# Gardlin/PCR-CG

Hardware: AMD Instinct MI355X
Metric: fragment-pairs/s KPFCNN+GCN fwd, 30k-pt pairs (higher is better)
Workload: dtype f32

## Files before the change

include/pcrcg.h:

```cpp
#ifndef PCRCG_H
#define PCRCG_H

#include <stddef.h>
#include <stdint.h>

#ifdef __cplusplus
extern "C" {
#endif

#define PCRCG_OK 0
#define PCRCG_EBADARG (-1)
#define PCRCG_EWORKSPACE (-2)
#define PCRCG_ELAUNCH (-3)
#define PCRCG_ECAPACITY (-4)

#define PCRCG_KPOINTS 15

const char* pcrcg_last_error(void);
#define PCRCG_ABI_VERSION 4
int pcrcg_abi_version(void);

int pcrcg_debug_set(const char* spec);
int pcrcg_debug_release(void);

// ... 6 lines not shown
int pcrcg_umap_order(const uint64_t* keys, int m, int* order, void* ws, size_t ws_bytes, void* stream);

size_t pcrcg_cellgrid_ws_bytes(int ns, int nb);
int pcrcg_cellgrid_build(const float* sup, int ns, const int* slen, int nb, float radius, void* grid,
                         size_t grid_bytes, void* stream);
int pcrcg_radius_query(const float* q, int nq, const int* qlen, int ns, const int* slen, int nb,
                       float radius, const void* grid, int cols, int64_t* out_idx, int* out_count,
                       int* out_max_count, int* status, void* stream);
int pcrcg_radius_query_ex(const float* q, int nq, const int* qlen, int ns, const int* slen, int nb,
                          float radius, const void* grid, int cols, int64_t* out_idx, int* out_count,
                          int* out_max_count, int* status, int* out_tie_rows, int* out_tie_count, void* stream);
int pcrcg_radius_query_groups(const float* q, int nq, const int* qlen, int ns, const int* slen, int nb, int group,
                              float radius, const void* grid, int cols, int64_t* out_idx, int* out_count,
                              int* out_max_count, int* status, int* out_tie_rows, int* out_tie_count, void* stream);
int pcrcg_radius_query_cells(const void* qgrid, const float* q, int nq, const int* qlen, const void* sgrid, int ns,
                             const int* slen, int nb, int group, float radius, int cols, int64_t* out_idx, int* out_count,
                             int* out_max_count, int* status, int* out_tie_rows, int* out_tie_count, void* stream);
size_t pcrcg_radius_neighbors_ws_bytes(int ns, int nb);
int pcrcg_radius_neighbors_batch(const float* q, int nq, const float* sup, int ns, const int* qlen,
                                 const int* slen, int nb, float radius, int cols, int64_t* out_idx,
                                 int* out_count, int* out_max_count, int* status, void* ws,
                                 size_t ws_bytes, void* stream);

#define PCRCG_MAX_REORDER_JOBS 12
typedef struct pcrcg_reorder_job {
    const float* q;
    const int* qlen;
    const int* rows;
    const int* count;
    int64_t* idx;
    int nq, nbq, cloud0, nrows, max_count, cols;
    float radius;
    int group;
    const float* sup;
    const void* forest;
    int forest_ns, forest_nb;
} pcrcg_reorder_job;
size_t pcrcg_kdforest_ws_bytes(int ns, int nb);
int pcrcg_kdforest_build(const float* sup, int ns, const int* slen, int nb, void* forest, size_t forest_bytes,
                         void* stream);
int pcrcg_radius_reorder(const float* q, int nq, const int* qlen, int nbq, const float* sup, int ns, int nb,
                         const void* forest, int cloud0, float radius, const int* rows, int nrows, const int* count,
                         int max_count, int cols, int64_t* idx, int* status, void* stream);
int pcrcg_radius_reorder_jobs(const pcrcg_reorder_job* jobs, int njobs, const float* sup, int ns, int nb,
                              const void* forest, int* status, void* stream);

size_t pcrcg_kpconv_ws_bytes(int ns);
int pcrcg_kpconv_aggregate(const float* q_pts, int nq, const float* s_pts, int ns, const int64_t* idx,
                           int h, int ld_idx, const float* x, int cin, const float* kp, float extent,
                           float* wf, float* inv_n, void* ws, size_t ws_bytes, void* stream);
int pcrcg_kpconv_aggregate_bf16(const float* q_pts, int nq, const float* s_pts, int ns, const int64_t* idx, int h,
                                int ld_idx, const float* x, int cin, const float* kp, float extent, void* x_bf16,
                                void* wf_bf16, float* inv_n, void* ws, size_t ws_bytes, void* stream);

void pcrcg_profile_kpconv(int enable);
int pcrcg_profile_kpconv_read(float* ms, int* nq, int* h, int* cin, int* cout, int* kind, int cap);

int pcrcg_gemm_f32(const float* a, int lda, const float* b, int ldb, int trans_b, float* c, int ldc, int m,
                   int n, int k, const float* row_scale, const float* bias, void* stream);
size_t pcrcg_gemm_colstats_bytes(int m, int n);
int pcrcg_gemm_f32_colstats(const float* a, int lda, const float* b, int ldb, int trans_b, float* c, int ldc,
                            int m, int n, int k, const float* row_scale, const float* bias, void* colstats,
                            size_t colstats_bytes, int* h_chunks, void* stream);
int pcrcg_gemm_bf16a_f32_colstats(const void* a_bf16, int lda, const float* b, int ldb, float* c, int ldc, int m, int n,
                                  int k, const float* row_scale, const float* bias, void* colstats,
                                  size_t colstats_bytes, int* h_chunks, void* stream);

int pcrcg_gemm_f32_fused(const float* a, int lda, const int64_t* idx, int ld_idx, int ns, const float* zero_row,
                         const void* a_sums, double a_count, float a_eps, float a_slope, const float* b, int ldb,
                         const float* bias, float* c, int ldc, int m, int n, int k, int accumulate, void* stream);

void pcrcg_gemm_set_mode(int mode);
int pcrcg_gemm_get_mode(void);
int pcrcg_gemm_redo_counts(unsigned long long* out2, int reset);
void pcrcg_thread_shares_gpu(int on);

int pcrcg_gather_max(const float* x, int ns, int c, const int64_t* idx, int nq, int h, int ld_idx,
                     float* out, void* stream);
int pcrcg_gather_first(const float* x, int ns, int c, const int64_t* idx, int nq, int ld_idx, float* out,
                       int ld_out, void* stream);
size_t pcrcg_instnorm_ws_bytes(int c);
int pcrcg_instnorm_stats_from_partials(const void* partials, int chunks, int c, double count, float eps,
                                       float* stats, void* stream);
int pcrcg_instnorm_stats(const float* x, int n, int c, int ldx, float eps, float* stats, void* ws,
                         size_t ws_bytes, void* stream);
int pcrcg_instnorm_apply(const float* x, int n, int c, int ldx, const float* stats, const float* res,
                         int ldr, const float* res_stats, float slope, float* y, int ldy, void* stream);
int pcrcg_instnorm_colsums(const float* x, int n, int c, int ldx, void* sums, void* stream);
int pcrcg_instnorm_apply_sums(const float* x, int n, int c, int ldx, const void* sums, double count, float eps,
                              const float* res, int ldr, const void* res_sums, float slope, float* y, int ldy,
                              void* stream);

int pcrcg_fill2d(float* dst, int ld, int rows, int cols, float value, void* stream);
int pcrcg_inject_image_features(const float* fmap, int c, int h, int w, const float* valid, const int64_t* inds2d,
                                const int64_t* inds3d, int n, long row_offset, long n_rows, float* x, int ldx,
                                void* stream);

typedef struct pcrcg_image_frame {
    const float* fmap;
    const float* depth;
    const float* valid;
    float world2camera[16];
    float intrinsics[16];
    float thresh;
    int h, w;
    int depth_h, depth_w;
// ... 191 lines not shown
```

pcrcg_amd/_lib.py:

```python
import ctypes
import os

_HERE = os.path.dirname(os.path.abspath(__file__))
LIB_PATH = os.path.join(_HERE, "libpcrcg_hip.so")


def lib_identity():
    import hashlib
    with open(LIB_PATH, "rb") as f:
        return LIB_PATH, hashlib.sha256(f.read()).hexdigest()[:16]

ABI_VERSION = 4

c_int, c_float, c_void_p, c_size_t = ctypes.c_int, ctypes.c_float, ctypes.c_void_p, ctypes.c_size_t

SIGNATURES = {
    "pcrcg_last_error": (ctypes.c_char_p, []),
    "pcrcg_abi_version": (c_int, []),
    "pcrcg_debug_set": (c_int, [ctypes.c_char_p]),
    "pcrcg_check_status": (c_int, [c_void_p, c_void_p]),
    "pcrcg_grid_subsample_ws_bytes": (c_size_t, [c_int, c_int]),
    "pcrcg_grid_subsample_batch": (c_int, [c_void_p, c_int, c_void_p, c_int, c_float, c_int, c_void_p, c_void_p,
                                           c_void_p, c_void_p, c_size_t, c_void_p]),
    "pcrcg_umap_order_ws_bytes": (c_size_t, [c_int]),
    "pcrcg_umap_order": (c_int, [c_void_p, c_int, c_void_p, c_void_p, c_size_t, c_void_p]),
    "pcrcg_cellgrid_ws_bytes": (c_size_t, [c_int, c_int]),
    "pcrcg_cellgrid_build": (c_int, [c_void_p, c_int, c_void_p, c_int, c_float, c_void_p, c_size_t, c_void_p]),
    "pcrcg_radius_query": (c_int, [c_void_p, c_int, c_void_p, c_int, c_void_p, c_int, c_float, c_void_p, c_int,
                                   c_void_p, c_void_p, c_void_p, c_void_p, c_void_p]),
    "pcrcg_radius_query_ex": (c_int, [c_void_p, c_int, c_void_p, c_int, c_void_p, c_int, c_float, c_void_p, c_int,
                                      c_void_p, c_void_p, c_void_p, c_void_p, c_void_p, c_void_p, c_void_p]),
    "pcrcg_radius_query_groups": (c_int, [c_void_p, c_int, c_void_p, c_int, c_void_p, c_int, c_int, c_float, c_void_p, c_int,
                                          c_void_p, c_void_p, c_void_p, c_void_p, c_void_p, c_void_p, c_void_p]),
    "pcrcg_radius_query_cells": (c_int, [c_void_p, c_void_p, c_int, c_void_p, c_void_p, c_int, c_void_p, c_int, c_int, c_float,
                                         c_int, c_void_p, c_void_p, c_void_p, c_void_p, c_void_p, c_void_p, c_void_p]),
    "pcrcg_kdforest_ws_bytes": (c_size_t, [c_int, c_int]),
    "pcrcg_kdforest_build": (c_int, [c_void_p, c_int, c_void_p, c_int, c_void_p, c_size_t, c_void_p]),
    "pcrcg_radius_reorder": (c_int, [c_void_p, c_int, c_void_p, c_int, c_void_p, c_int, c_int, c_void_p, c_int,
                                     c_float, c_void_p, c_int, c_void_p, c_int, c_int, c_void_p, c_void_p, c_void_p]),
    "pcrcg_radius_reorder_jobs": (c_int, [c_void_p, c_int, c_void_p, c_int, c_int, c_void_p, c_void_p, c_void_p]),
    "pcrcg_radius_neighbors_ws_bytes": (c_size_t, [c_int, c_int]),
    "pcrcg_radius_neighbors_batch": (c_int, [c_void_p, c_int, c_void_p, c_int, c_void_p, c_void_p, c_int, c_float,
                                             c_int, c_void_p, c_void_p, c_void_p, c_void_p, c_void_p, c_size_t,
                                             c_void_p]),
    "pcrcg_kpconv_ws_bytes": (c_size_t, [c_int]),
    "pcrcg_kpconv_aggregate": (c_int, [c_void_p, c_int, c_void_p, c_int, c_void_p, c_int, c_int, c_void_p, c_int,
                                       c_void_p, c_float, c_void_p, c_void_p, c_void_p, c_size_t, c_void_p]),
    "pcrcg_kpconv_aggregate_bf16": (c_int, [c_void_p, c_int, c_void_p, c_int, c_void_p, c_int, c_int, c_void_p, c_int,
                                            c_void_p, c_float, c_void_p, c_void_p, c_void_p, c_void_p, c_size_t,
                                            c_void_p]),
    "pcrcg_profile_kpconv": (None, [c_int]),
    "pcrcg_profile_kpconv_read": (c_int, [c_void_p, c_void_p, c_void_p, c_void_p, c_void_p, c_void_p, c_int]),
    "pcrcg_gemm_f32": (c_int, [c_void_p, c_int, c_void_p, c_int, c_int, c_void_p, c_int, c_int, c_int, c_int,
                               c_void_p, c_void_p, c_void_p]),
    "pcrcg_gemm_colstats_bytes": (c_size_t, [c_int, c_int]),
    "pcrcg_gemm_f32_colstats": (c_int, [c_void_p, c_int, c_void_p, c_int, c_int, c_void_p, c_int, c_int, c_int, c_int,
                                        c_void_p, c_void_p, c_void_p, c_size_t, c_void_p, c_void_p]),
    "pcrcg_gemm_bf16a_f32_colstats": (c_int, [c_void_p, c_int, c_void_p, c_int, c_void_p, c_int, c_int, c_int, c_int,
                                              c_void_p, c_void_p, c_void_p, c_size_t, c_void_p, c_void_p]),
    "pcrcg_gemm_f32_fused": (c_int, [c_void_p, c_int, c_void_p, c_int, c_int, c_void_p, c_void_p, ctypes.c_double, c_float,
                                     c_float, c_void_p, c_int, c_void_p, c_void_p, c_int, c_int, c_int, c_int, c_int, c_void_p]),
    "pcrcg_gemm_set_mode": (None, [c_int]),
    "pcrcg_gemm_get_mode": (c_int, []),
    "pcrcg_gemm_redo_counts": (c_int, [c_void_p, c_int]),
    "pcrcg_instnorm_stats_from_partials": (c_int, [c_void_p, c_int, c_int, ctypes.c_double, c_float, c_void_p,
                                                   c_void_p]),
    "pcrcg_gather_max": (c_int, [c_void_p, c_int, c_int, c_void_p, c_int, c_int, c_int, c_void_p, c_void_p]),
    "pcrcg_gather_first": (c_int, [c_void_p, c_int, c_int, c_void_p, c_int, c_int, c_void_p, c_int, c_void_p]),
    "pcrcg_instnorm_ws_bytes": (c_size_t, [c_int]),
    "pcrcg_instnorm_stats": (c_int, [c_void_p, c_int, c_int, c_int, c_float, c_void_p, c_void_p, c_size_t, c_void_p]),
    "pcrcg_instnorm_apply": (c_int, [c_void_p, c_int, c_int, c_int, c_void_p, c_void_p, c_int, c_void_p, c_float,
                                     c_void_p, c_int, c_void_p]),
    "pcrcg_instnorm_colsums": (c_int, [c_void_p, c_int, c_int, c_int, c_void_p, c_void_p]),
    "pcrcg_instnorm_apply_sums": (c_int, [c_void_p, c_int, c_int, c_int, c_void_p, ctypes.c_double, c_float, c_void_p, c_int,
                                          c_void_p, c_float, c_void_p, c_int, c_void_p]),
    "pcrcg_fill2d": (c_int, [c_void_p, c_int, c_int, c_int, c_float, c_void_p]),
    "pcrcg_inject_image_features": (c_int, [c_void_p, c_int, c_int, c_int, c_void_p, c_void_p, c_void_p, c_int, ctypes.c_long,
                                            ctypes.c_long, c_void_p, c_int, c_void_p]),
    "pcrcg_project_depth_ws_bytes": (c_size_t, [c_int]),
    "pcrcg_project_depth": (c_int, [c_void_p, c_int, c_void_p, c_int, c_int, c_void_p, c_void_p, c_float, c_void_p, c_void_p,
                                    c_void_p, c_void_p, c_size_t, c_void_p]),
    "pcrcg_inject_frames": (c_int, [c_void_p, ctypes.c_long, ctypes.c_long, c_void_p, c_int, c_int, c_void_p, c_int, c_void_p]),
    "pcrcg_superglue_valid_maps": (c_int, [c_void_p, c_int, c_void_p, c_int, c_void_p, c_void_p, c_int, c_int, c_int, c_void_p,
                                           c_void_p, c_void_p]),
    "pcrcg_knn": (c_int, [c_void_p, c_int, c_int, c_void_p, c_void_p]),
    "pcrcg_edgeconv_ws_bytes": (c_size_t, [c_int]),
    "pcrcg_edgeconv_reduce": (c_int, [c_void_p, c_int, c_void_p, c_int, c_void_p, c_int, c_int, c_int, c_float,
                                      c_void_p, c_int, c_void_p, c_void_p, c_size_t, c_void_p]),
    "pcrcg_edgeconv_reduce_sums": (c_int, [c_void_p, c_int, c_void_p, c_int, c_void_p, c_int, c_int, c_int, c_void_p, c_int,
                                           c_void_p, c_void_p]),
    "pcrcg_softmax_rows": (c_int, [c_void_p, c_int, c_int, c_int, c_float, c_void_p]),
    "pcrcg_attention_supported": (c_int, [c_int]),
    "pcrcg_attention": (c_int, [c_void_p, c_int, c_void_p, c_int, c_void_p, c_int, c_void_p, c_int, c_int, c_int, c_int,
                                c_int, c_float, c_void_p]),
    "pcrcg_softmax_matvec": (c_int, [c_void_p, c_int, c_int, c_int, c_float, c_void_p, c_int, c_void_p, c_int, c_void_p]),
    "pcrcg_copy2d": (c_int, [c_void_p, c_int, c_void_p, c_int, c_int, c_int, c_void_p]),
    "pcrcg_add": (c_int, [c_void_p, c_void_p, c_void_p, ctypes.c_long, c_void_p]),
    "pcrcg_l2norm_rows": (c_int, [c_void_p, c_int, c_void_p, c_int, c_int, c_int, c_void_p]),
    "pcrcg_sigmoid_scores": (c_int, [c_void_p, c_int, c_void_p, c_int, c_void_p]),
    "pcrcg_kpfcnn_ws_bytes": (c_size_t, [c_void_p, c_void_p]),
    "pcrcg_kpfcnn_group_ws_bytes": (c_size_t, [c_void_p, c_void_p, c_int]),
    "pcrcg_kpfcnn_forward_group": (c_int, [c_void_p, c_void_p, c_void_p, c_int, c_void_p, c_size_t, c_void_p]),
    "pcrcg_kpfcnn_forward": (c_int, [c_void_p, c_void_p, c_void_p, c_void_p, c_size_t, c_void_p]),
# ... 111 lines not shown
```

pcrcg_amd/csrc/common.h:

```cpp
#pragma once
#include <hip/hip_runtime.h>

#include <cstdarg>
#include <cstdint>
#include <cstdio>
#include <mutex>

#include "pcrcg.h"

namespace pcrcg {

void set_error(const char* fmt, ...);

inline hipStream_t as_stream(void* s) { return reinterpret_cast<hipStream_t>(s); }

struct Carver {
    char* base;
    size_t cap;
    size_t off = 0;
    Carver(void* ws, size_t bytes) : base(static_cast<char*>(ws)), cap(bytes) {}
    template <typename T>
    T* take(size_t count) {
        size_t bytes = (count * sizeof(T) + 255) & ~size_t(255);
        T* p = reinterpret_cast<T*>(base + off);
// ... 20 lines not shown
void gemm_x6_release_det();
void trainops_release_det();
void conv2d_release_det();

int kdforest_build_levels(const float* sup, int ns, const int* slen, int nb, int per_level, const int* level_base, void* forest,
                          size_t forest_bytes, hipStream_t stream);

int radius_fast_cap();
int radius_query_pass(const float* q, int nq, const int* qlen, int ns, const int* slen, int nb, int group, float radius,
                      const void* grid, int cols, int64_t* out_idx, int* out_count, int* out_max_count, int* status,
                      int* out_tie_rows, int* out_tie_count, hipStream_t st, int pass);

bool gemm_x6_shared();
void gemm_x6_set_shared(int on);
int radius_cells_pass(const void* qgrid, const float* q, int nq, const int* qlen, const void* sgrid, int ns, const int* slen,
                      int nb, int group, float radius, int cols, int64_t* out_idx, int* out_count, int* out_max_count,
                      int* status, int* out_tie_rows, int* out_tie_count, hipStream_t st, int pass);
constexpr int kRadiusRedoStatus = 4;

struct GemmExtra {
    const long long* a_idx = nullptr;
    int a_idx_ld = 0, a_ns = 0;
    const float* a_zero = nullptr;
    bool accumulate = false;
    const double* a_sums = nullptr;
    double a_count = 0.0;
    float a_eps = 1e-5f, a_slope = 1.0f;
    int grad_operand = 0;
};

struct GemmPair {
    const float* a = nullptr;
    float* c = nullptr;
    int m = 0;
    const float* row_scale = nullptr;
    void* colstats = nullptr;
    int* h_chunks = nullptr;
    bool c_zeroed = false;
    const long long* a_idx = nullptr;
    int a_ns = 0;
    const double* a_sums = nullptr;
    double a_count = 0.0;
};
struct GemmGroup {
    int n = 0;
    GemmPair p[3];
};

int kpconv_pack(const float* x, int ns, int cin, const float* s_pts, void* ws, size_t ws_bytes, hipStream_t st,
                unsigned short* x_bf16 = nullptr);
int kpconv_aggregate_rows(const float* q_pts, int nq, const float* s_pts, int ns, const int64_t* idx, int h, int ld_idx,
                          const float* x, int cin, const float* kp, float extent, float* wf, float* inv_n, void* ws,
                          size_t ws_bytes, hipStream_t st, bool pack, bool stream_out, int c1_ld = 0);
int kpconv_aggregate_bf16(const float* q_pts, int nq, const float* s_pts, int ns, const int64_t* idx, int h, int ld_idx,
                          const float* x, unsigned short* x_bf16, int cin, const float* kp, float extent,
                          unsigned short* wf_bf16, float* inv_n, void* ws, size_t ws_bytes, hipStream_t st);

struct NormJob {
    const float* x; const double* sums; const float* res; const double* res_sums; float* y;
    const float* s_pts; float4* pk;
    int n; double count;
    float* stats_out = nullptr;
};
int instnorm_apply_sums_multi(const NormJob* jobs, int count, int c, int ldx, float eps, int ldr, float slope, int ldy, bool pack,
                              hipStream_t st);

struct GatherJob { const float* x; const int64_t* idx; float* out; int ns, nq, h, ld_idx; };
int gather_max_multi(const GatherJob* jobs, int count, int c, hipStream_t st);
int heads_multi(const float* const* x, const int* rows, int count, int ld, int fd, float* const* feats, float* const* s_ov,
                float* const* s_sal, hipStream_t st);
int copy2d_multi(const float* const* src, float* const* dst, const int* rows, int count, int ld_src, int ld_dst, int cols,
                 hipStream_t st);
int instnorm_colsums_multi(const float* const* x, double* const* sums, const int* n, int count, int c, int ldx, hipStream_t st);

struct EdgeCloud {
    const float* ctr; const float* nbr; const int* idx; float* emax; double* sums; int n, k;
};
bool edgeconv_rows_ok(const EdgeCloud* cl, int count, int ld_ctr, int ld_nbr, int ld_emax, int c);
int edgeconv_rows_multi(const EdgeCloud* cl, int count, int ld_ctr, int ld_nbr, int ld_emax, int c, bool atomic, int* nchunks_out,
                        hipStream_t st);

struct AttnCloud { const float* q; const float* k; const float* v; float* out; int n, ms; };
bool attention_mfma_ok(const AttnCloud* cl, int count, int ldq, int ldk, int ldv, int d);
int attention_mfma_multi(const AttnCloud* cl, int count, int ldq, int ldk, int ldv, int ldo, int heads, int d, float scale,
                         hipStream_t st);
bool attention_bwd_mfma_ok(int n, int ms, int d, int ldq, int ldk, int ldv, int ld_do);
int attention_bwd_mfma(const float* q, int ldq, const float* k, int ldk, const float* v, int ldv, const float* o, int ldo,
                       const float* d_o, int ld_do, float* dq, int ld_dq, float* dk, int ld_dk, float* dv, int ld_dv, int n, int ms,
                       int heads, int d, float scale, hipStream_t st);

struct DebugOpts {
    int stat_sums = 1;
    int stat_sums_rows = 1 << 30;
    int att_mfma = 1;
    int radius_blocks = 0;
    int kd_blocks = 0;
    int att_tq = 16;
    int kd_spin_limit = 0;
    int gemm_log = 0;
    int x6_tile = -1, x6_splitk = 0, x6_t1 = 1, x6_t2 = 1, x6_order = -1, x6_big = 0, x6_h2 = 1;
    int train_side_stream = 1;
    int gemm_tile = -1, gemm_splitk = 0, gemm_split_target = 768;
    int deterministic = 0;
    int bwd_mfma = 1;
};
const DebugOpts& debug_opts();
// ... 63 lines not shown
```

pcrcg_amd/csrc/kpconv.hip:

```cpp
#include <mutex>
#include <vector>

#include <hip/hip_ext.h>

#include "common.h"

namespace pcrcg {

struct ProfRec { hipEvent_t a, b; int nq, h, cin, cout, kind; };
static int g_prof_on = 0;
static std::vector<ProfRec> g_prof;
static std::mutex g_prof_mu;

KpProfScope::KpProfScope(hipStream_t s, int nq_, int h_, int cin_, int cout_, int kind_)
    : st(s), a(nullptr), b(nullptr), nq(nq_), h(h_), cin(cin_), cout(cout_), kind(kind_),
      on((g_prof_on & (kind_ == 3 ? 2 : kind_ == 4 ? 4 : 1)) != 0) {
    if (!on) return;
    (void)hipEventCreate(&a);
    (void)hipEventCreate(&b);
}
KpProfScope::~KpProfScope() {
    if (!on) return;
    std::lock_guard<std::mutex> lock(g_prof_mu);
    g_prof.push_back({a, b, nq, h, cin, cout, kind});
// ... 183 lines not shown
    float kpx[K], kpy[K], kpz[K];
#pragma unroll
    for (int k = 0; k < K; ++k) { kpx[k] = kp[3 * k]; kpy[k] = kp[3 * k + 1]; kpz[k] = kp[3 * k + 2]; }
    const float inv_extent = 1.0f / extent;
    const float qx = q_pts[3 * (long)q], qy = q_pts[3 * (long)q + 1], qz = q_pts[3 * (long)q + 2];
    float acc[K];
#pragma unroll
    for (int k = 0; k < K; ++k) acc[k] = 0.f;
    int npos = 0;
    const long long* row = idx + (long)q * ld_idx;
    for (int h0 = 0; h0 < H; h0 += C1_PARTS * C1_BATCH) {
        long long iv[C1_BATCH];
#pragma unroll
        for (int b = 0; b < C1_BATCH; ++b) {
            const int h = h0 + b * C1_PARTS + part;
            iv[b] = row[h < H ? h : H - 1];
        }
        float nx[C1_BATCH], ny[C1_BATCH], nz[C1_BATCH], xv[C1_BATCH];
#pragma unroll
        for (int b = 0; b < C1_BATCH; ++b) {
            const int h = h0 + b * C1_PARTS + part;
            const bool real = h < H && iv[b] >= 0 && iv[b] < ns;
            const long ic = real ? iv[b] : 0;
            const float4 p = pk[ic];
            nx[b] = p.x - qx;
            ny[b] = p.y - qy;
            nz[b] = p.z - qz;
            const float v = p.w;
            xv[b] = real ? v : 0.f;
        }
#pragma unroll
        for (int b = 0; b < C1_BATCH; ++b) {
            npos += xv[b] > 0.0f ? 1 : 0;
#pragma unroll
            for (int k = 0; k < K; ++k) {
                const float dx = nx[b] - kpx[k], dy = ny[b] - kpy[k], dz = nz[b] - kpz[k];
                acc[k] = fmaf(fmaxf(1.0f - __builtin_amdgcn_sqrtf(dx * dx + dy * dy + dz * dz) * inv_extent, 0.0f),
                              xv[b], acc[k]);
            }
        }
    }
#pragma unroll
    for (int d = 1; d < C1_PARTS; d <<= 1) {
#pragma unroll
        for (int k = 0; k < K; ++k) acc[k] += __shfl_xor(acc[k], d, 64);
        npos += __shfl_xor(npos, d, 64);
    }
    if (qraw >= nq) return;
#pragma unroll
    for (int k = 0; k < K; ++k)
        if ((k & (C1_PARTS - 1)) == part) wf[(long)q * ld_wf + k] = acc[k];
    if (ld_wf > K && part == C1_PARTS - 1) wf[(long)q * ld_wf + K] = 0.f;
    if (part == 0) inv_n[q] = 1.0f / (float)(npos > 1 ? npos : 1);
}

__global__ void __launch_bounds__(kWavesPerBlock * 64) k_kpconv_generic(
    const float* __restrict__ q_pts, int nq, const float* __restrict__ s_pts, int ns,
    const long long* __restrict__ idx, int H, int ld_idx, const float* __restrict__ x, int cin,
    const float* __restrict__ kp, float extent, const unsigned char* __restrict__ pos, float* __restrict__ wf,
    float* __restrict__ inv_n) {
    __shared__ __attribute__((aligned(16))) float s_w[kWavesPerBlock][64][16];
    __shared__ int s_idx[kWavesPerBlock][64];
    const int lane = threadIdx.x & 63, wave = threadIdx.x >> 6;
    const int gw = blockIdx.x * kWavesPerBlock + wave, nw = gridDim.x * kWavesPerBlock;
    const float inv_extent = 1.0f / extent;
    for (int q = gw; q < nq; q += nw) {
        const float qx = q_pts[3 * (long)q], qy = q_pts[3 * (long)q + 1], qz = q_pts[3 * (long)q + 2];
        int npos = 0;
        for (int cbase = 0; cbase < cin; cbase += 64) {
            float acc[K];
#pragma unroll
            for (int k = 0; k < K; ++k) acc[k] = 0.0f;
            for (int hc = 0; hc < H; hc += 64) {
                const int h = hc + lane;
                int i = -1;
                if (h < H) {
                    const long long v = idx[(long)q * ld_idx + h];
                    i = (v >= 0 && v < ns) ? (int)v : -1;
                }
                __builtin_amdgcn_wave_barrier();
                if (i >= 0) {
                    const float nx = s_pts[3 * (long)i] - qx, ny = s_pts[3 * (long)i + 1] - qy,
                                nz = s_pts[3 * (long)i + 2] - qz;
                    for (int k = 0; k < K; ++k) {
                        const float dx = nx - kp[3 * k], dy = ny - kp[3 * k + 1], dz = nz - kp[3 * k + 2];
                        s_w[wave][lane][k] = fmaxf(1.0f - sqrtf(dx * dx + dy * dy + dz * dz) * inv_extent, 0.0f);
                    }
                }
                s_idx[wave][lane] = i;
                if (cbase == 0) npos += __popcll(__ballot(i >= 0 && pos[i >= 0 ? i : 0] != 0));
                __builtin_amdgcn_wave_barrier();
                const int hn = H - hc < 64 ? H - hc : 64;
                const int c = cbase + lane;
                for (int hh = 0; hh < hn; ++hh) {
                    const int ii = s_idx[wave][hh];
                    if (ii < 0) continue;
                    const float xv = c < cin ? x[(long)ii * cin + c] : 0.0f;
#pragma unroll
                    for (int k = 0; k < K; ++k) acc[k] = fmaf(s_w[wave][hh][k], xv, acc[k]);
                }
            }
            const int c = cbase + lane;
            if (c < cin)
#pragma unroll
                for (int k = 0; k < K; ++k) wf[(long)q * K * cin + (long)k * cin + c] = acc[k];
        }
// ... 10 lines not shown
    return cv.ok() ? pk : nullptr;
}

int kpconv_pack(const float* x, int ns, int cin, const float* s_pts, void* ws, size_t ws_bytes, hipStream_t st,
                unsigned short* x_bf16) {
    Carver cv(ws, ws_bytes);
    unsigned char* pos = cv.take<unsigned char>((size_t)ns + 1);
    float4* pk = cv.take<float4>((size_t)ns + 1);
    PCRCG_CHECK_WS(cv);
    if (ns > 0) hipLaunchKernelGGL(k_row_positive, dim3((ns + 3) / 4), dim3(256), 0, st, x, ns, cin, s_pts, pos, pk, x_bf16);
    PCRCG_CHECK_LAUNCH();
    return PCRCG_OK;
}

}

using namespace pcrcg;

extern "C" {

void pcrcg_profile_kpconv(int enable) {
    std::lock_guard<std::mutex> lock(g_prof_mu);
    for (auto& r : g_prof) { (void)hipEventDestroy(r.a); (void)hipEventDestroy(r.b); }
    g_prof.clear();
    g_prof_on = enable;
}

int pcrcg_profile_kpconv_read(float* ms, int* nq, int* h, int* cin, int* cout, int* kind, int cap) {
    std::lock_guard<std::mutex> lock(g_prof_mu);
    int n = 0;
    for (auto& r : g_prof) {
        if (n >= cap) break;
        if (hipEventSynchronize(r.b) != hipSuccess) return -1;
        float t = 0.f;
        if (hipEventElapsedTime(&t, r.a, r.b) != hipSuccess) return -1;
        ms[n] = t; nq[n] = r.nq; h[n] = r.h; cin[n] = r.cin; cout[n] = r.cout; kind[n] = r.kind;
        ++n;
    }
    return n;
}

size_t pcrcg_kpconv_ws_bytes(int ns) {
    const size_t n = (size_t)(ns > 0 ? ns : 0) + 1;
    return carve_bytes(n, 1) + carve_bytes(n, sizeof(float4));
}

int pcrcg_kpconv_aggregate(const float* q_pts, int nq, const float* s_pts, int ns, const int64_t* idx,
                           int h, int ld_idx, const float* x, int cin, const float* kp, float extent,
                           float* wf, float* inv_n, void* ws, size_t ws_bytes, void* stream) {
    return kpconv_aggregate_rows(q_pts, nq, s_pts, ns, idx, h, ld_idx, x, cin, kp, extent, wf, inv_n, ws, ws_bytes,
                                 as_stream(stream), true, true, 0);
}

int pcrcg_kpconv_aggregate_bf16(const float* q_pts, int nq, const float* s_pts, int ns, const int64_t* idx, int h,
                                int ld_idx, const float* x, int cin, const float* kp, float extent, void* x_bf16,
                                void* wf_bf16, float* inv_n, void* ws, size_t ws_bytes, void* stream) {
    return kpconv_aggregate_bf16(q_pts, nq, s_pts, ns, idx, h, ld_idx, x, static_cast<unsigned short*>(x_bf16), cin, kp,
                                 extent, static_cast<unsigned short*>(wf_bf16), inv_n, ws, ws_bytes, as_stream(stream));
}
}

namespace pcrcg {

int kpconv_aggregate_rows(const float* q_pts, int nq, const float* s_pts, int ns, const int64_t* idx, int h, int ld_idx,
                          const float* x, int cin, const float* kp, float extent, float* wf, float* inv_n, void* ws,
                          size_t ws_bytes, hipStream_t st, bool pack, bool stream_out, int c1_ld) {
    PCRCG_CHECK_ARG(nq >= 0 && ns >= 0 && h >= 1 && ld_idx >= h && cin >= 1 && (c1_ld == 0 || c1_ld == K || c1_ld == K + 1));
    PCRCG_CHECK_ARG(extent > 0.0f);
    if (nq == 0) return PCRCG_OK;
    PCRCG_CHECK_ARG(q_pts && s_pts && idx && x && kp && wf && inv_n && ws);
    PCRCG_CHECK_ARG(ns >= 1);
    Carver cv(ws, ws_bytes);
    unsigned char* pos = cv.take<unsigned char>((size_t)ns + 1);
    float4* pk = cv.take<float4>((size_t)ns + 1);
    PCRCG_CHECK_WS(cv);
    const long long* idx_ll = reinterpret_cast<const long long*>(idx);
    const int max_blocks = 256 * 32;
    auto blocks_for = [&](long waves) {
        long b = (waves + kWavesPerBlock - 1) / kWavesPerBlock;
        return (int)(b > max_blocks ? max_blocks : b);
    };
    if (cin == 1) {
        if (pack) hipLaunchKernelGGL(k_pack_c1, dim3((ns + 255) / 256), dim3(256), 0, st, x, ns, s_pts, pk);
        KpProfScope prof_scope(st, nq, h, cin, 0, 0);
        hipExtLaunchKernelGGL(k_kpconv_c1, dim3((int)(((long)nq * C1_PARTS + 255) / 256)), dim3(256), 0, st, prof_scope.a,
                              prof_scope.b, 0, q_pts, nq, s_pts, ns, idx_ll, h, ld_idx, (const float4*)pk, kp, extent, wf,
                              inv_n, c1_ld > 0 ? c1_ld : K);
        PCRCG_CHECK_LAUNCH();
        return PCRCG_OK;
    }
    if (pack && ns > 0)
        hipLaunchKernelGGL(k_row_positive, dim3((ns + 3) / 4), dim3(256), 0, st, x, ns, cin, s_pts, pos, pk,
                           (unsigned short*)nullptr);
    KpProfScope prof_scope(st, nq, h, cin, 0, 0);
    const bool aligned = (cin % 4 == 0) && ((reinterpret_cast<uintptr_t>(x) & 15) == 0) &&
                         ((reinterpret_cast<uintptr_t>(wf) & 15) == 0);
    if (!aligned) {
        hipLaunchKernelGGL(k_kpconv_generic, dim3(blocks_for(nq)), dim3(kWavesPerBlock * 64), 0, st, q_pts, nq, s_pts,
                           ns, idx_ll, h, ld_idx, x, cin, kp, extent, pos, wf, inv_n);
        PCRCG_CHECK_LAUNCH();
        return PCRCG_OK;
    }
    if (cin == 68 || cin == 132) {
        const int blocks = blocks_for((long)nq);
#define LAUNCH_T(NBV, NT)                                                                                                        \
        hipExtLaunchKernelGGL((k_kpconv_mfma<NBV, NT, float, true>), dim3(blocks), dim3(kWavesPerBlock * 64), 0, st, prof_scope.a, \
                              prof_scope.b, 0, q_pts, nq, s_pts, ns, idx_ll, h, ld_idx, x, cin, kp, extent,                      \
                              (const float4*)pk, wf, inv_n, 1)
        if (cin == 132) { if (stream_out) LAUNCH_T(2, true); else LAUNCH_T(2, false); }
        else { if (stream_out) LAUNCH_T(1, true); else LAUNCH_T(1, false); }
#undef LAUNCH_T
        PCRCG_CHECK_LAUNCH();
        return PCRCG_OK;
    }
    const int nblk = (cin + 63) / 64;
    int nb = nblk >= 4 ? 4 : (nblk >= 2 ? 2 : 1);
    while (nb > 1 && ((long)nq * ((nblk + nb - 1) / nb) < 16384 || nblk % nb != 0)) nb >>= 1;
    const int nchunk = (nblk + nb - 1) / nb;
    const int blocks = blocks_for((long)nq * nchunk);
#define LAUNCH(NBV, NT)                                                                                                 \
    hipExtLaunchKernelGGL((k_kpconv_mfma<NBV, NT, float>), dim3(blocks), dim3(kWavesPerBlock * 64), 0, st, prof_scope.a, \
                          prof_scope.b, 0, q_pts, nq, s_pts, ns, idx_ll, h, ld_idx, x, cin, kp, extent,                 \
                          (const float4*)pk, wf, inv_n, nchunk)
    if (stream_out) {
        if (nb == 4) LAUNCH(4, true);
        else if (nb == 2) LAUNCH(2, true);
        else LAUNCH(1, true);
    } else {
        if (nb == 4) LAUNCH(4, false);
        else if (nb == 2) LAUNCH(2, false);
        else LAUNCH(1, false);
    }
#undef LAUNCH
    PCRCG_CHECK_LAUNCH();
    return PCRCG_OK;
}

int kpconv_aggregate_bf16(const float* q_pts, int nq, const float* s_pts, int ns, const int64_t* idx, int h, int ld_idx,
                          const float* x, unsigned short* x_bf16, int cin, const float* kp, float extent,
                          unsigned short* wf_bf16, float* inv_n, void* ws, size_t ws_bytes, hipStream_t st) {
    PCRCG_CHECK_ARG(nq >= 0 && ns >= 1 && h >= 1 && ld_idx >= h && cin >= 4 && cin % 4 == 0 && extent > 0.0f);
    if (nq == 0) return PCRCG_OK;
    PCRCG_CHECK_ARG(q_pts && s_pts && idx && x && x_bf16 && kp && wf_bf16 && inv_n && ws);
    PCRCG_CHECK_ARG((reinterpret_cast<uintptr_t>(x_bf16) & 7) == 0 && (reinterpret_cast<uintptr_t>(wf_bf16) & 7) == 0);
    PCRCG_PROPAGATE(kpconv_pack(x, ns, cin, s_pts, ws, ws_bytes, st, x_bf16));
    Carver cv(ws, ws_bytes);
    cv.take<unsigned char>((size_t)ns + 1);
    float4* pk = cv.take<float4>((size_t)ns + 1);
    const long long* idx_ll = reinterpret_cast<const long long*>(idx);
    const int nblk = (cin + 63) / 64;
    int nb = nblk >= 4 ? 4 : (nblk >= 2 ? 2 : 1);
    while (nb > 1 && ((long)nq * ((nblk + nb - 1) / nb) < 16384 || nblk % nb != 0)) nb >>= 1;
    const int nchunk = (nblk + nb - 1) / nb;
    long blocks = ((long)nq * nchunk + kWavesPerBlock - 1) / kWavesPerBlock;
    if (blocks > 256 * 32) blocks = 256 * 32;
    KpProfScope prof_scope(st, nq, h, cin, 0, 2);
#define LAUNCHB(NBV)                                                                                                      \
    hipExtLaunchKernelGGL((k_kpconv_mfma<NBV, true, unsigned short>), dim3((int)blocks), dim3(kWavesPerBlock * 64), 0, st, \
                          prof_scope.a, prof_scope.b, 0, q_pts, nq, s_pts, ns, idx_ll, h, ld_idx, x_bf16, cin, kp, extent, \
                          (const float4*)pk, wf_bf16, inv_n, nchunk)
    if (nb == 4) LAUNCHB(4);
    else if (nb == 2) LAUNCHB(2);
    else LAUNCHB(1);
#undef LAUNCHB
    PCRCG_CHECK_LAUNCH();
    return PCRCG_OK;
}

}
```

pcrcg_amd/csrc/runner.hip:

```cpp
#include <vector>

#include <cstdlib>

#include "common.h"

namespace pcrcg {
bool gemm_bt_accumulates(int m, int n, int k, long m_total = 0);
int gemm_bt_colstats(const float* a, int lda, const float* b, int ldb, float* c, int ldc, int m, int n, int k,
                     const float* row_scale, const float* bias, void* colstats, size_t colstats_bytes, int* h_chunks,
                     hipStream_t st, bool c_zeroed, bool colstats_sums = false);
int gemm_bf16a_bt_colstats(const void* a_bf16, int lda, const float* b, int ldb, float* c, int ldc, int m, int n, int k,
                           const float* row_scale, const float* bias, void* colstats, size_t colstats_bytes,
                           int* h_chunks, hipStream_t st, bool c_zeroed, bool colstats_sums);
bool gemm_colstats_sums_ok();
bool gemm_extra_ok();
int gemm_bt_extra(const float* a, int lda, const float* b, int ldb, float* c, int ldc, int m, int n, int k, hipStream_t st,
                  bool c_zeroed, const GemmExtra& ex, const float* bias = nullptr, void* colstats = nullptr,
                  size_t colstats_bytes = 0, int* h_chunks = nullptr, bool colstats_sums = false);
bool gemm_pair_ok();
int gemm_bt_colstats_pair(const float* a, int lda, const float* b, int ldb, float* c, int ldc, int m, int n, int k,
                          const float* row_scale, const float* bias, void* colstats, size_t colstats_bytes, int* h_chunks,
                          hipStream_t st, bool c_zeroed, bool colstats_sums, const GemmGroup* grp);
int gemm_bt_extra_pair(const float* a, int lda, const float* b, int ldb, float* c, int ldc, int m, int n, int k, hipStream_t st,
                       bool c_zeroed, const GemmExtra& ex, const float* bias, void* colstats, size_t colstats_bytes,
// ... 254 lines not shown
            q.m = m_of(g);
            q.colstats = st ? st->partials[g] : nullptr;
            q.h_chunks = st ? &st->chunks[g] : nullptr;
            q.c_zeroed = c_zeroed;
            if (tabs) { q.a_idx = reinterpret_cast<const long long*>(tabs[g]->idx); q.a_ns = a.rows[g]; }
            if (a_sums) { q.a_sums = static_cast<const double*>(a_sums->partials[g]); q.a_count = (double)a.rows[g]; }
        }
        c.check(gemm_bt_extra_pair(a.p[0], a.ld, w, ldw, y.p[0], y.ld, m_of(0), y.cols, a.cols, c.st, c_zeroed, ex, bias,
                                   st ? st->partials[0] : nullptr, st ? st->bytes : 0, st ? &st->chunks[0] : nullptr,
                                   st && st->sums, &p));
        return;
    }
    for (int g = 0; g < c.G; ++g) {
        GemmExtra ex = extra(g);
        c.check(gemm_bt_extra(a.p[g], a.ld, w, ldw, y.p[g], y.ld, m_of(g), y.cols, a.cols, c.st, c_zeroed, ex, bias,
                              st ? st->partials[g] : nullptr, st ? st->bytes : 0, st ? &st->chunks[g] : nullptr, st && st->sums));
    }
}

bool lazy_stats_ready(Ctx& c, const Mat& x, Stat* xs) {
    if (!xs || !xs->sums || x.ld % 4 != 0 || x.cols > 4096) return false;
    fill_sums(c, x, xs);
    return true;
}
bool linear_norm(Ctx& c, const Mat& x, Stat* xs, float slope, const float* w, int ldw, const float* bias, const Mat& y,
                 Stat* st = nullptr) {
    if (!gemm_extra_ok() || !lazy_stats_ready(c, x, xs)) return false;
    linear_extra(c, x, w, ldw, bias, y, 0, nullptr, nullptr, xs, slope, false, y.zeroed, st);
    return true;
}

struct Batches { const pcrcg_batch* b[GMAX]; };

int kp_cin(const pcrcg_block& blk, const Mat& x) { return (blk.kp_w_pad && blk.cin_pad > x.cols) ? blk.cin_pad : x.cols; }
const float* kp_weight(const pcrcg_block& blk, const Mat& x) {
    return (blk.kp_w_pad && blk.cin_pad > 0 && kp_cin(blk, x) == blk.cin_pad) ? blk.kp_w_pad : blk.kp_w;
}

void kpconv(Ctx& c, const Batches& B, const pcrcg_block& blk, const Mat& x, const Mat& y, Stat* st = nullptr,
            void* const* packed_ws = nullptr) {
    const int l = blk.layer;
    const size_t m = c.mark();
    Mat xin = x;
    const float* const w = kp_weight(blk, x);
    const int cin = kp_cin(blk, x);
    if (cin > x.cols) {
        xin = c.mat(x.rows, cin);
        if (c.live())
            for (int g = 0; g < c.G; ++g) {
                c.check(hipMemsetAsync(xin.p[g], 0, sizeof(float) * (size_t)x.rows[g] * cin, c.st) == hipSuccess ? PCRCG_OK
                                                                                                                   : PCRCG_ELAUNCH);
                c.check(pcrcg_copy2d(x.p[g], x.ld, xin.p[g], cin, x.rows[g], x.cols, c.st));
            }
    }
    int nq[GMAX], ns[GMAX];
    const float* q[GMAX];
    const pcrcg_table* tab[GMAX];
    float* inv_n[GMAX];
    void* ws[GMAX];
    size_t wsb[GMAX];
    for (int g = 0; g < c.G; ++g) {
        const pcrcg_batch& b = *B.b[g];
        tab[g] = blk.strided ? &b.pools[l] : &b.neighbors[l];
        q[g] = blk.strided ? b.points[l + 1] : b.points[l];
        nq[g] = blk.strided ? b.n_points[l + 1] : b.n_points[l];
        ns[g] = b.n_points[l];
        inv_n[g] = static_cast<float*>(c.raw(sizeof(float) * (nq[g] > 0 ? nq[g] : 1)));
        wsb[g] = pcrcg_kpconv_ws_bytes(ns[g]);
        ws[g] = (packed_ws && packed_ws[g]) ? packed_ws[g] : c.raw(wsb[g]);
    }
    const bool c1_16 = cin == 1 && blk.kp_wt != nullptr;
    const float* const kp_wt = blk.kp_wt;
    const int kk = c1_16 ? 16 : PCRCG_KPOINTS * cin;
    if (c.bf16 && kp_wt && cin % 32 == 0) {
        for (int g = 0; g < c.G; ++g) {
            const pcrcg_batch& b = *B.b[g];
            void* xb = c.raw(sizeof(unsigned short) * (size_t)(ns[g] > 0 ? ns[g] : 1) * cin);
            void* wfb = c.raw(sizeof(unsigned short) * (size_t)(nq[g] > 0 ? nq[g] : 1) * kk);
            if (c.live()) {
                c.check(pcrcg_kpconv_aggregate_bf16(q[g], nq[g], b.points[l], ns[g], tab[g]->idx, tab[g]->cols, tab[g]->ld, xin.p[g],
                                                    cin, blk.kp, blk.extent, xb, wfb, inv_n[g], ws[g], wsb[g], c.st));
                c.check(gemm_bf16a_bt_colstats(wfb, kk, kp_wt, kk, y.p[g], y.ld, nq[g], y.cols, kk, inv_n[g], nullptr,
                                               st ? st->partials[g] : nullptr, st ? st->bytes : 0, st ? &st->chunks[g] : nullptr,
                                               c.st, y.zeroed, st && st->sums));
            }
        }
        c.release(m);
        return;
    }
    Mat wf = c.mat(nq, kk);
    if (c.live()) {
        for (int g = 0; g < c.G; ++g) {
            const pcrcg_batch& b = *B.b[g];
            if (c1_16)
                c.check(kpconv_aggregate_rows(q[g], nq[g], b.points[l], ns[g], tab[g]->idx, tab[g]->cols, tab[g]->ld, xin.p[g], cin,
                                              blk.kp, blk.extent, wf.p[g], inv_n[g], ws[g], wsb[g], c.st, true,
                                              true, 16));
            else if (packed_ws && packed_ws[g] && xin.p[g] == x.p[g])
                c.check(kpconv_aggregate_rows(q[g], nq[g], b.points[l], ns[g], tab[g]->idx, tab[g]->cols, tab[g]->ld, xin.p[g], cin,
                                              blk.kp, blk.extent, wf.p[g], inv_n[g], ws[g], wsb[g], c.st, false,
                                              true));
            else
                c.check(pcrcg_kpconv_aggregate(q[g], nq[g], b.points[l], ns[g], tab[g]->idx, tab[g]->cols, tab[g]->ld, xin.p[g], cin,
                                               blk.kp, blk.extent, wf.p[g], inv_n[g], ws[g], wsb[g], c.st));
        }
        if (kp_wt)
// ... 577 lines not shown
```

Baseline: 596.1.

## Fuse single-channel KPConv aggregation with weight GEMM and column stats

Adds a kernel for cin==1 KPConv layers that computes kernel-point influence sums per query, keeps them in shared memory, then multiplies by the 15xcout weights and writes outputs while accumulating per-column sum and sum-of-squares for instance norm. This replaces the separate aggregation write, GEMM launch and stats pass, avoiding the intermediate buffer round trip and extra launches for the first layer. It adds a partials-to-sums reduction kernel when sums are requested and restricts the path to cout shapes that divide 256.

```diff
diff --git a/include/pcrcg.h b/include/pcrcg.h
--- a/include/pcrcg.h
+++ b/include/pcrcg.h
@@ -82,6 +82,11 @@
 int pcrcg_kpconv_aggregate_bf16(const float* q_pts, int nq, const float* s_pts, int ns, const int64_t* idx, int h,
                                 int ld_idx, const float* x, int cin, const float* kp, float extent, void* x_bf16,
                                 void* wf_bf16, float* inv_n, void* ws, size_t ws_bytes, void* stream);
+
+int pcrcg_kpconv_c1_fused(const float* q_pts, int nq, const float* s_pts, int ns, const int64_t* idx, int h, int ld_idx,
+                          const float* x, const float* kp, float extent, const float* kp_w, int cout, float* out, int ld_out,
+                          void* colstats, size_t colstats_bytes, int colstats_sums, int* h_chunks, void* ws, size_t ws_bytes,
+                          void* stream);
 
 void pcrcg_profile_kpconv(int enable);
 int pcrcg_profile_kpconv_read(float* ms, int* nq, int* h, int* cin, int* cout, int* kind, int cap);
diff --git a/pcrcg_amd/_lib.py b/pcrcg_amd/_lib.py
--- a/pcrcg_amd/_lib.py
+++ b/pcrcg_amd/_lib.py
@@ -49,6 +49,9 @@
     "pcrcg_kpconv_aggregate_bf16": (c_int, [c_void_p, c_int, c_void_p, c_int, c_void_p, c_int, c_int, c_void_p, c_int,
                                             c_void_p, c_float, c_void_p, c_void_p, c_void_p, c_void_p, c_size_t,
                                             c_void_p]),
+    "pcrcg_kpconv_c1_fused": (c_int, [c_void_p, c_int, c_void_p, c_int, c_void_p, c_int, c_int, c_void_p, c_void_p, c_float,
+                                      c_void_p, c_int, c_void_p, c_int, c_void_p, c_size_t, c_int, c_void_p, c_void_p, c_size_t,
+                                      c_void_p]),
     "pcrcg_profile_kpconv": (None, [c_int]),
     "pcrcg_profile_kpconv_read": (c_int, [c_void_p, c_void_p, c_void_p, c_void_p, c_void_p, c_void_p, c_int]),
     "pcrcg_gemm_f32": (c_int, [c_void_p, c_int, c_void_p, c_int, c_int, c_void_p, c_int, c_int, c_int, c_int,
diff --git a/pcrcg_amd/csrc/common.h b/pcrcg_amd/csrc/common.h
--- a/pcrcg_amd/csrc/common.h
+++ b/pcrcg_amd/csrc/common.h
@@ -96,6 +96,11 @@
 int kpconv_aggregate_rows(const float* q_pts, int nq, const float* s_pts, int ns, const int64_t* idx, int h, int ld_idx,
                           const float* x, int cin, const float* kp, float extent, float* wf, float* inv_n, void* ws,
                           size_t ws_bytes, hipStream_t st, bool pack, bool stream_out, int c1_ld = 0);
+bool kpconv_c1_fused_ok(int cout, int ld_out);
+int kpconv_c1_fused(const float* q_pts, int nq, const float* s_pts, int ns, const int64_t* idx, int h, int ld_idx, const float* x,
+                    const float* kp, float extent, const float* w, int w_sk, int w_sc, int cout, float* out, int ld_out,
+                    void* colstats, size_t colstats_bytes, bool colstats_sums, int* h_chunks, void* ws, size_t ws_bytes,
+                    hipStream_t st);
 int kpconv_aggregate_bf16(const float* q_pts, int nq, const float* s_pts, int ns, const int64_t* idx, int h, int ld_idx,
                           const float* x, unsigned short* x_bf16, int cin, const float* kp, float extent,
                           unsigned short* wf_bf16, float* inv_n, void* ws, size_t ws_bytes, hipStream_t st);
diff --git a/pcrcg_amd/csrc/kpconv.hip b/pcrcg_amd/csrc/kpconv.hip
--- a/pcrcg_amd/csrc/kpconv.hip
+++ b/pcrcg_amd/csrc/kpconv.hip
@@ -259,6 +259,132 @@
         if ((k & (C1_PARTS - 1)) == part) wf[(long)q * ld_wf + k] = acc[k];
     if (ld_wf > K && part == C1_PARTS - 1) wf[(long)q * ld_wf + K] = 0.f;
     if (part == 0) inv_n[q] = 1.0f / (float)(npos > 1 ? npos : 1);
+}
+
+__global__ void __launch_bounds__(256) k_kpconv_c1_fused(
+    const float* __restrict__ q_pts, int nq, const float* __restrict__ s_pts, int ns, const long long* __restrict__ idx, int H,
+    int ld_idx, const float4* __restrict__ pk, const float* __restrict__ kp, float extent, const float* __restrict__ w, int w_sk,
+    int w_sc, int cout, float* __restrict__ out, int ld_out, double* __restrict__ colp, int colp_chunks) {
+    __shared__ __attribute__((aligned(16))) float s_s[64][16];
+    __shared__ double s_red[8][256];
+    const int tid = threadIdx.x;
+    {
+        const int t = blockIdx.x * 256 + tid;
+        const int part = t & (C1_PARTS - 1);
+        const int qraw = t / C1_PARTS;
+        const int q = qraw < nq ? qraw : nq - 1;
+        float kpx[K], kpy[K], kpz[K];
+#pragma unroll
+        for (int k = 0; k < K; ++k) { kpx[k] = kp[3 * k]; kpy[k] = kp[3 * k + 1]; kpz[k] = kp[3 * k + 2]; }
+        const float inv_extent = 1.0f / extent;
+        const float qx = q_pts[3 * (long)q], qy = q_pts[3 * (long)q + 1], qz = q_pts[3 * (long)q + 2];
+        float acc[K];
+#pragma unroll
+        for (int k = 0; k < K; ++k) acc[k] = 0.f;
+        int npos = 0;
+        const long long* row = idx + (long)q * ld_idx;
+        for (int h0 = 0; h0 < H; h0 += C1_PARTS * C1_BATCH) {
+            long long iv[C1_BATCH];
+#pragma unroll
+            for (int b = 0; b < C1_BATCH; ++b) {
+                const int h = h0 + b * C1_PARTS + part;
+                iv[b] = row[h < H ? h : H - 1];
+            }
+            bool any_real = false;
+#pragma unroll
+            for (int b = 0; b < C1_BATCH; ++b) any_real = any_real || (h0 + b * C1_PARTS + part < H && iv[b] >= 0 && iv[b] < ns);
+            if (__ballot(any_real) == 0ull) continue;
+            float nx[C1_BATCH], ny[C1_BATCH], nz[C1_BATCH], xv[C1_BATCH];
+#pragma unroll
+            for (int b = 0; b < C1_BATCH; ++b) {
+                const int h = h0 + b * C1_PARTS + part;
+                const bool real = h < H && iv[b] >= 0 && iv[b] < ns;
+                const long ic = real ? iv[b] : 0;
+                const float4 p = pk[ic];
+                nx[b] = p.x - qx;
+                ny[b] = p.y - qy;
+                nz[b] = p.z - qz;
+                xv[b] = real ? p.w : 0.f;
+            }
+#pragma unroll
+            for (int b = 0; b < C1_BATCH; ++b) {
+                npos += xv[b] > 0.0f ? 1 : 0;
+#pragma unroll
+                for (int k = 0; k < K; ++k) {
+                    const float dx = nx[b] - kpx[k], dy = ny[b] - kpy[k], dz = nz[b] - kpz[k];
+                    acc[k] = fmaf(fmaxf(1.0f - __builtin_amdgcn_sqrtf(dx * dx + dy * dy + dz * dz) * inv_extent, 0.0f),
+                                  xv[b], acc[k]);
+                }
+            }
+        }
+#pragma unroll
+        for (int d = 1; d < C1_PARTS; d <<= 1) {
+#pragma unroll
+            for (int k = 0; k < K; ++k) acc[k] += __shfl_xor(acc[k], d, 64);
+            npos += __shfl_xor(npos, d, 64);
+        }
+        const int lr = tid / C1_PARTS;
+#pragma unroll
+        for (int k = 0; k < K; ++k)
+            if ((k & (C1_PARTS - 1)) == part) s_s[lr][k] = acc[k];
+        if (part == C1_PARTS - 1) s_s[lr][K] = 1.0f / (float)(npos > 1 ? npos : 1);
+    }
+    __syncthreads();
+    const int c4 = cout >> 2, cg = tid % c4, rstep = 256 / c4;
+    float4 wr[K];
+#pragma unroll
+    for (int k = 0; k < K; ++k) {
+        const float* p = w + (long)k * w_sk + (long)(4 * cg) * w_sc;
+        wr[k] = make_float4(p[0], p[w_sc], p[2 * (long)w_sc], p[3 * (long)w_sc]);
+    }
+    double sum[4] = {0.0, 0.0, 0.0, 0.0}, sq[4] = {0.0, 0.0, 0.0, 0.0};
+    for (int r = tid / c4; r < 64; r += rstep) {
+        const long gq = (long)blockIdx.x * 64 + r;
+        if (gq >= nq) break;
+        float sv[16];
+#pragma unroll
+        for (int i = 0; i < 4; ++i) {
+            const float4 t4 = *reinterpret_cast<const float4*>(&s_s[r][4 * i]);
+            sv[4 * i] = t4.x; sv[4 * i + 1] = t4.y; sv[4 * i + 2] = t4.z; sv[4 * i + 3] = t4.w;
+        }
+        float4 o = make_float4(0.f, 0.f, 0.f, 0.f);
+#pragma unroll
+        for (int k = 0; k < K; ++k) {
+            o.x = fmaf(sv[k], wr[k].x, o.x);
+            o.y = fmaf(sv[k], wr[k].y, o.y);
+            o.z = fmaf(sv[k], wr[k].z, o.z);
+            o.w = fmaf(sv[k], wr[k].w, o.w);
+        }
+        o.x *= sv[K]; o.y *= sv[K]; o.z *= sv[K]; o.w *= sv[K];
+        *reinterpret_cast<float4*>(out + gq * ld_out + 4 * cg) = o;
+        sum[0] += (double)o.x; sq[0] += (double)o.x * (double)o.x;
+        sum[1] += (double)o.y; sq[1] += (double)o.y * (double)o.y;
+        sum[2] += (double)o.z; sq[2] += (double)o.z * (double)o.z;
+        sum[3] += (double)o.w; sq[3] += (double)o.w * (double)o.w;
+    }
+    if (!colp) return;
+#pragma unroll
+    for (int j = 0; j < 4; ++j) { s_red[j][tid] = sum[j]; s_red[4 + j][tid] = sq[j]; }
+    __syncthreads();
+    if (tid >= c4) return;
+#pragma unroll
+    for (int j = 0; j < 8; ++j) {
+        double a = s_red[j][tid];
+        for (int g = 1; g < rstep; ++g) a += s_red[j][tid + g * c4];
+        const long col = (j < 4 ? 0 : cout) + 4 * cg + (j & 3);
+        if (colp_chunks < 0) unsafeAtomicAdd(&colp[col], a);
+        else colp[col * colp_chunks + blockIdx.x] = a;
+    }
+}
+
+__global__ void __launch_bounds__(256) k_partials_to_sums(const double* __restrict__ part, int rows, int chunks, double* __restrict__ sums) {
+    const int lane = threadIdx.x & 63, j = blockIdx.x * 4 + (threadIdx.x >> 6);
+    if (j >= rows) return;
+    double a = 0.0;
+    for (int c = lane; c < chunks; c += 64) a += part[(long)j * chunks + c];
+#pragma unroll
+    for (int d = 32; d >= 1; d >>= 1) a += __shfl_xor(a, d, 64);
+    if (lane == 0) sums[j] += a;
 }
 
 __global__ void __launch_bounds__(kWavesPerBlock * 64) k_kpconv_generic(
@@ -375,6 +501,14 @@
                                  as_stream(stream), true, true, 0);
 }
 
+int pcrcg_kpconv_c1_fused(const float* q_pts, int nq, const float* s_pts, int ns, const int64_t* idx, int h, int ld_idx,
+                          const float* x, const float* kp, float extent, const float* kp_w, int cout, float* out, int ld_out,
+                          void* colstats, size_t colstats_bytes, int colstats_sums, int* h_chunks, void* ws, size_t ws_bytes,
+                          void* stream) {
+    return kpconv_c1_fused(q_pts, nq, s_pts, ns, idx, h, ld_idx, x, kp, extent, kp_w, cout, 1, cout, out, ld_out, colstats,
+                           colstats_bytes, colstats_sums != 0, h_chunks, ws, ws_bytes, as_stream(stream));
+}
+
 int pcrcg_kpconv_aggregate_bf16(const float* q_pts, int nq, const float* s_pts, int ns, const int64_t* idx, int h,
                                 int ld_idx, const float* x, int cin, const float* kp, float extent, void* x_bf16,
                                 void* wf_bf16, float* inv_n, void* ws, size_t ws_bytes, void* stream) {
@@ -455,6 +589,44 @@
         else LAUNCH(1, false);
     }
 #undef LAUNCH
+    PCRCG_CHECK_LAUNCH();
+    return PCRCG_OK;
+}
+
+bool kpconv_c1_fused_ok(int cout, int ld_out) {
+    return cout >= 4 && cout % 4 == 0 && 256 % (cout / 4) == 0 && ld_out >= cout && ld_out % 4 == 0;
+}
+int kpconv_c1_fused(const float* q_pts, int nq, const float* s_pts, int ns, const int64_t* idx, int h, int ld_idx, const float* x,
+                    const float* kp, float extent, const float* w, int w_sk, int w_sc, int cout, float* out, int ld_out,
+                    void* colstats, size_t colstats_bytes, bool colstats_sums, int* h_chunks, void* ws, size_t ws_bytes,
+                    hipStream_t st) {
+    if (h_chunks) *h_chunks = 0;
+    PCRCG_CHECK_ARG(nq >= 0 && ns >= 0 && h >= 1 && ld_idx >= h && extent > 0.0f && ld_out >= cout && w_sk >= 1 && w_sc >= 1);
+    if (nq == 0) return PCRCG_OK;
+    PCRCG_CHECK_ARG(q_pts && s_pts && idx && x && kp && w && out && ws && ns >= 1);
+    Carver cv(ws, ws_bytes);
+    cv.take<unsigned char>((size_t)ns + 1);
+    float4* pk = cv.take<float4>((size_t)ns + 1);
+    PCRCG_CHECK_WS(cv);
+    double* const spill = cv.take<double>(2 * (size_t)cout * ((nq + 63) / 64));
+    const bool two_pass = colstats && h_chunks && colstats_sums && cv.ok();
+    PCRCG_CHECK_ARG(kpconv_c1_fused_ok(cout, ld_out) && (reinterpret_cast<uintptr_t>(out) & 15) == 0);
+    const int blocks = (nq + 63) / 64;
+    double* colp = nullptr;
+    int chunks = 0;
+    if (colstats && h_chunks) {
+        if (colstats_sums) chunks = -1;
+        else if (carve_bytes(2 * (size_t)cout * blocks, sizeof(double)) <= colstats_bytes) chunks = blocks;
+        if (chunks != 0) colp = static_cast<double*>(colstats);
+        *h_chunks = chunks;
+    }
+    hipLaunchKernelGGL(k_pack_c1, dim3((ns + 255) / 256), dim3(256), 0, st, x, ns, s_pts, pk);
+    KpProfScope prof_scope(st, nq, h, 1, cout, 0);
+    hipExtLaunchKernelGGL(k_kpconv_c1_fused, dim3(blocks), dim3(256), 0, st, prof_scope.a, prof_scope.b, 0, q_pts, nq, s_pts, ns,
+                          reinterpret_cast<const long long*>(idx), h, ld_idx, (const float4*)pk, kp, extent, w, w_sk, w_sc, cout, out, ld_out,
+                          two_pass ? spill : colp, two_pass ? blocks : chunks);
+    if (two_pass)
+        hipLaunchKernelGGL(k_partials_to_sums, dim3((2 * cout + 3) / 4), dim3(256), 0, st, spill, 2 * cout, blocks, colp);
     PCRCG_CHECK_LAUNCH();
     return PCRCG_OK;
 }
diff --git a/pcrcg_amd/csrc/runner.hip b/pcrcg_amd/csrc/runner.hip
--- a/pcrcg_amd/csrc/runner.hip
+++ b/pcrcg_amd/csrc/runner.hip
@@ -330,6 +330,23 @@
                                                                                                                    : PCRCG_ELAUNCH);
                 c.check(pcrcg_copy2d(x.p[g], x.ld, xin.p[g], cin, x.rows[g], x.cols, c.st));
             }
+    }
+    if (cin == 1 && (blk.kp_w || blk.kp_wt) && gemm_pair_ok() && kpconv_c1_fused_ok(y.cols, y.ld)) {
+        for (int g = 0; g < c.G; ++g) {
+            const pcrcg_batch& b = *B.b[g];
+            const pcrcg_table& t = blk.strided ? b.pools[l] : b.neighbors[l];
+            const int rows = blk.strided ? b.n_points[l + 1] : b.n_points[l];
+            const size_t wsb = pcrcg_kpconv_ws_bytes(b.n_points[l]) + carve_bytes(2 * (size_t)y.cols * ((rows + 63) / 64), sizeof(double));
+            void* const ws = c.raw(wsb);
+            if (c.live())
+                c.check(kpconv_c1_fused(blk.strided ? b.points[l + 1] : b.points[l], blk.strided ? b.n_points[l + 1] : b.n_points[l],
+                                        b.points[l], b.n_points[l], t.idx, t.cols, t.ld, xin.p[g], blk.kp, blk.extent,
+                                        blk.kp_w ? blk.kp_w : blk.kp_wt, blk.kp_w ? y.cols : 1, blk.kp_w ? 1 : 16, y.cols, y.p[g], y.ld,
+                                        st ? st->partials[g] : nullptr, st ? st->bytes : 0, st && st->sums, st ? &st->chunks[g] : nullptr,
+                                        ws, wsb, c.st));
+        }
+        c.release(m);
+        return;
     }
     int nq[GMAX], ns[GMAX];
     const float* q[GMAX];
```

Result: no change. 594.7 (-0.2%).
